# p-sawicki/entropy_coding

Hardware: AMD Instinct MI355X
Metric: Mbins/s encode+decode, intra QP32 synthetic bin buffers (higher is better)
Workload: dtype u32

## Files before the change

### entropy_coding_amd/csrc/cabac_kernels_v4.hip

```cpp
#include <cstdlib>
#include <type_traits>

#include "cabac_device.h"
#include "cabac_kernels.h"
#include "cabac_quad.h"

namespace cabac {


struct QuadEnc {
  uint64_t low;
  uint32_t range;
  int32_t pend;
  uint32_t buf;
  int32_t nbuf;
  uint32_t pos;
  uint8_t *dst;
  uint32_t cap;
};

__device__ __forceinline__ void quad_put_byte(QuadEnc &e, uint32_t byte, bool writer) {
  if (writer && e.pos < e.cap) e.dst[e.pos] = (uint8_t)byte;
  e.pos += 1;
}
// ... 117 lines not shown
    quad_put_byte(e, held, writer);
    held = 0;
    nb = 0;
  }
  const uint32_t n_bits = e.pos * 8u + nb;
  if (nb) quad_put_byte(e, held, writer);
  return n_bits;
}

template <class... Sets>
__global__ __launch_bounds__(64) void encode_kernel_v4(uint32_t n_sub, const cabac_substream_desc *__restrict__ desc,
                                                       const uint16_t *__restrict__ records, uint8_t *__restrict__ bytes,
                                                       cabac_substream_result *__restrict__ results, Sets... sets) {
  constexpr bool kSets = sizeof...(Sets) != 0;
  __shared__ uint32_t ctx[kQuadSubs * kQuadCtxStride];
  const uint32_t lane = threadIdx.x, row = lane >> 4, j = lane & 15u;
  const uint32_t sub = blockIdx.x * kQuadSubs + row;
  const QuadSetUse su = quad_set_use(sub, sub < n_sub, sets...);
  const bool live = sub < n_sub && !su.bad;
  const cabac_substream_desc d = desc[live ? sub : 0];
  const uint32_t n = live ? d.n_records : 0u;
  const uint16_t *rec = records + d.rec_offset;
  uint32_t *rctx = ctx + row * kQuadCtxStride;
  if constexpr (kSets) quad_ctx_load<true>(rctx, d.qp, d.init_id & 3u, j, 16u, su, sets...);
  else quad_ctx_init(rctx, d.qp, d.init_id & 3u, j);
  __syncthreads();

  QuadEnc e;
  e.low = 0;
  e.range = 510;
  e.pend = 0;
  e.buf = 0;
  e.nbuf = 0;
  e.pos = 0;
  e.dst = bytes + d.byte_offset;
  e.cap = live ? d.byte_capacity : 0u;
  const bool writer = live && j == 0;
  uint32_t bad = 0;

  uint32_t next_rec = j < n ? rec[j] : 0;
  for (uint32_t base = 0; __ballot(base < n) != 0; base += 16) {
    const uint32_t r = next_rec;
    const uint32_t info = quad_phase_a(r, base + j < n, lane, row, rctx, bad);
    const QuadEncInfo f = quad_unpack(info);
    {
      const uint32_t nxt = base + 16u + j;
      next_rec = nxt < n ? rec[nxt] : 0;
    }
    if (__ballot(info >> 12) == 0) quad_enc_steps<false, false>(f, e, writer, QuadPost());
    else quad_enc_steps<true, false>(f, e, writer, QuadPost());
  }

  const uint32_t n_bits = live ? quad_enc_finish(e, (d.init_id & CABAC_SUB_ALIGN_RBSP) != 0, writer, (d.init_id & CABAC_SUB_PROBE) != 0) : 0u;
  const uint64_t bad_mask = __ballot(bad != 0);
  const bool row_bad = ((bad_mask >> (row * 16u)) & 0xffffull) != 0;
  if (writer) {
    cabac_substream_result res;
    res.n_bits = n_bits;
    res.flags = (e.pos > e.cap ? CABAC_RES_OVERFLOW : 0u) | (row_bad ? CABAC_RES_BAD_RECORD : 0u);
    results[sub] = res;
  }
  if constexpr (kSets) {
    __syncthreads();
    quad_ctx_export(rctx, j, 16u, su, sets...);
    quad_bad_set_result(results, sub, j == 0, su);
  }
}

constexpr uint32_t kUnitSlots = 12;
constexpr uint32_t kUnitDump = 11;

template <int N>
__device__ __forceinline__ uint32_t row_shr(uint32_t v) {
  return (uint32_t)__builtin_amdgcn_update_dpp(0, (int)v, 0x110 + N, 0xf, 0xf, true);
}


struct QuadUnits {
  uint32_t m;
  uint64_t odd_rows;
  uint64_t store_lanes;
};

template <bool kHalfRows = false>
__device__ __forceinline__ QuadUnits quad_list_units(const QuadEnc &e, const uint32_t *plo, const uint32_t *phi,
                                                     const uint32_t *ppend, uint32_t row, uint32_t j, bool live,
                                                     uint32_t *list, uint32_t lane = 0) {
  const uint32_t c = (j & 3u) * kQuadSubs + row;
  const uint64_t low = ((uint64_t)phi[c] << 32) | plo[c];
  const uint32_t pend = ppend[c];
  const uint32_t nun = (pend >> 4) & neg_mask(j - 4u);
  const uint64_t v = low >> (9u + (pend & 15u));
  uint32_t incl = nun + row_shr<1>(nun);
  incl += row_shr<2>(incl);
  const uint32_t idx = incl - nun;
  const uint32_t first = (uint32_t)(v >> (((nun - 1u) & 1u) << 4));
  const uint32_t second = (uint32_t)v & 0xffffu;
  const uint32_t has1 = neg_mask(0u - nun);
  const uint32_t has2 = neg_mask(1u - nun);
  list[sel(has1, idx, kUnitDump)] = first;
  list[sel(has2, idx + 1u, kUnitDump)] = second;
  QuadUnits u;
  if (kHalfRows) u.m = (lane & 8u) ? row_bcast<11>(incl) : row_bcast<3>(incl);
  else u.m = row_bcast<3>(incl);
  const uint32_t room = e.cap - e.pos - 2u * u.m;
  const uint32_t rowodd = neg_mask(0u - u.m) & (neg_mask(0u - ((uint32_t)e.nbuf ^ 1u)) | neg_mask(room));
  u.odd_rows = __ballot(live && rowodd != 0);
  u.store_lanes = __ballot(live && j < u.m);
  return u;
}

__device__ __forceinline__ void quad_flush_list(QuadEnc &e, uint32_t m, const uint32_t *list, bool writer) {
  for (uint32_t k = 0; k < 8u && __ballot(k < m) != 0; k++) {
    if (k < m) quad_flush_lead(e, list[k], writer);
  }
}

__device__ __forceinline__ void quad_emit_units(QuadEnc &e, const QuadUnits &u, uint32_t j, const uint32_t *list,
                                                bool writer) {
  if (u.odd_rows != 0) return quad_flush_list(e, u.m, list, writer);
  const uint32_t act = neg_mask(j - u.m);
  const uint32_t jnz = neg_mask(0u - j);
  const uint32_t before = list[sel(act & jnz, j - 1u, kUnitDump)];
  const uint32_t mine = list[sel(act, j, kUnitDump)];
  const uint32_t last = list[sel(neg_mask(0u - u.m), u.m - 1u, kUnitDump)];
  const uint32_t x = (mine & 0x1ffffu) ^ 0xffffu;
  if (__ballot((act & neg_mask(x - 1u)) != 0) != 0) return quad_flush_list(e, u.m, list, writer);
  const uint32_t prev = sel(jnz, before & 0xffffu, e.buf);
  const uint32_t unit = prev + (mine >> 16);
  const uint32_t be = ((unit & 0xffu) << 8) | ((unit >> 8) & 0xffu);
  uint8_t *addr = e.dst + e.pos + 2u * j;
  uint64_t saved;
  asm volatile("s_mov_b64 %0, exec\n\ts_mov_b64 exec, %1\n\tglobal_store_short %2, %3, off\n\ts_mov_b64 exec, %0"
               : "=&s"(saved) : "s"(u.store_lanes), "v"(addr), "v"(be) : "memory");
  e.buf = sel(neg_mask(0u - u.m), last & 0xffffu, e.buf);
  e.pos += 2u * u.m;
}

#ifdef CABAC_V5_PROFILE
__device__ unsigned long long g_v5_prof[16];
#define V5_TICK(var) const unsigned long long var = __builtin_amdgcn_s_memtime()
#define V5_ADD(slot, t0, t1) \
  if (blockIdx.x == 0 && lane == 0) g_v5_prof[slot] += (t1) - (t0)
#else
#define V5_TICK(var)
#define V5_ADD(slot, t0, t1)
#endif
#ifndef CABAC_V5_STAMP_UNIT
#define CABAC_V5_STAMP_UNIT 0
#endif


struct QuadRngCap {
  uint32_t w[8];
};

template <int I, bool kAlign>
__device__ __forceinline__ void quad_rng_step(const QuadEncInfo &f, uint32_t &range, QuadRngCap &cap) {
  const uint32_t k = row_bcast<I>(f.k), c2 = row_bcast<I>(f.c2), lpsm = row_bcast<I>(f.lpsm);
  const uint32_t t = (__umul24((range >> 5) & 15u, k) + c2) >> 1;
  const uint32_t rm = range - t;
  const uint32_t x = sel(lpsm, t, rm);
  const uint32_t nb = (uint32_t)(__builtin_clz(x) - 23);
  range = x << nb;
  if (kAlign) range = sel(row_bcast<I>(f.alm), 256u, range);
  const uint32_t w = rm | (nb << 9);
  if (I & 1) cap.w[I >> 1] |= w << 16;
  else cap.w[I >> 1] = w;
}

struct QuadEncRow {
  uint32_t k[16], c2[16], lpsm[16];
};
template <int I, bool kAlign>
__device__ __forceinline__ void quad_rng_step_row(const QuadEncRow &u, const QuadEncInfo &f, uint32_t &range, QuadRngCap &cap) {
  const uint32_t t = (__umul24((range >> 5) & 15u, u.k[I]) + u.c2[I]) >> 1;
  const uint32_t rm = range - t;
  const uint32_t x = sel(u.lpsm[I], t, rm);
  const uint32_t nb = (uint32_t)(__builtin_clz(x) - 23);
  range = x << nb;
  if (kAlign) range = sel(row_bcast<I>(f.alm), 256u, range);
  const uint32_t w = rm | (nb << 9);
  if (I & 1) cap.w[I >> 1] |= w << 16;
  else cap.w[I >> 1] = w;
}
template <bool kAlign>
__device__ __forceinline__ void quad_rng_steps_row(const QuadEncRow &u, const QuadEncInfo &f, uint32_t &range, QuadRngCap &cap) {
#define QSTEP(I) quad_rng_step_row<I, kAlign>(u, f, range, cap)
  QSTEP(0); QSTEP(1); QSTEP(2); QSTEP(3); QSTEP(4); QSTEP(5); QSTEP(6); QSTEP(7);
  QSTEP(8); QSTEP(9); QSTEP(10); QSTEP(11); QSTEP(12); QSTEP(13); QSTEP(14); QSTEP(15);
#undef QSTEP
}

template <bool kAlign>
__device__ __forceinline__ void quad_rng_steps(const QuadEncInfo &f, uint32_t &range, QuadRngCap &cap) {
#define QSTEP(I) quad_rng_step<I, kAlign>(f, range, cap)
  QSTEP(0); QSTEP(1); QSTEP(2); QSTEP(3); QSTEP(4); QSTEP(5); QSTEP(6); QSTEP(7);
  QSTEP(8); QSTEP(9); QSTEP(10); QSTEP(11); QSTEP(12); QSTEP(13); QSTEP(14); QSTEP(15);
#undef QSTEP
}

__device__ __forceinline__ uint64_t shl64(uint32_t lo, uint32_t hi, uint32_t n) { return (((uint64_t)hi << 32) | lo) << n; }

__device__ __forceinline__ uint32_t quad_cap_mine(const QuadRngCap &cap, uint32_t j) {
  const uint32_t h = j >> 1;
  const uint32_t a0 = (h & 1u) ? cap.w[1] : cap.w[0], a1 = (h & 1u) ? cap.w[3] : cap.w[2], a2 = (h & 1u) ? cap.w[5] : cap.w[4],
                 a3 = (h & 1u) ? cap.w[7] : cap.w[6];
  const uint32_t b0 = (h & 2u) ? a1 : a0, b1 = (h & 2u) ? a3 : a2;
  const uint32_t pair = (h & 4u) ? b1 : b0;
  return ((j & 1u) ? pair >> 16 : pair) & 0xfffu;
}

__device__ __forceinline__ void quad_low_quads12(uint32_t w12, uint32_t info, uint32_t &v0, uint32_t &v1, uint32_t &s) {
  const uint32_t rm = w12 & 0x1ffu, nb = (w12 >> 9) & 7u;
  const uint32_t lpsm = bit_mask<9>(info), pem = bit_mask<11>(info), ep = (info >> 10) & 1u;
  const uint32_t term = ((rm & lpsm) << nb) | (rm & pem);
  s = nb + ep;
  uint64_t v = term;
  {
    const uint32_t p0 = row_shr<1>(term), ps = row_shr<1>(s);
    v = shl64(p0, 0u, s) + v;
    s += ps;
  }
  v0 = (uint32_t)v;
  {
    const uint32_t p0 = row_shr<2>(v0), ps = row_shr<2>(s);
    v = shl64(p0, 0u, s) + v;
    s += ps;
  }
// ... 225 lines not shown
    }
    if (n_iters != 0) {
#pragma unroll
      for (uint32_t h = 0; h < kSync; h++) list_step(kSync * (n_iters - 1u) + h);
    }
    if (j == 0u) {
      fin_acc[unit][row] = acc;
      fin_rem[unit][row] = rem;
    }
    __syncthreads();
    __syncthreads();
  } else {
    __builtin_amdgcn_s_setprio(CABAC_V6_PRIO_EMIT);
    QuadEnc e;
    e.low = 0;
    e.range = 0;
    e.pend = 0;
    e.buf = 0;
    e.nbuf = 0;
    e.pos = 0;
    e.dst = bytes + d.byte_offset;
    e.cap = live ? d.byte_capacity : 0u;
    const bool writer = live && j == 0;
    auto emit_step = [&](uint32_t step) {
      const uint32_t slot = step & (kRing - 1u);
      const uint32_t *list = unit_list[unit][slot][row];
      QuadUnits u;
      u.m = unit_count[unit][slot][row];
      const uint32_t room = e.cap - e.pos - 2u * u.m;
      const uint32_t rowodd = neg_mask(0u - u.m) & (neg_mask(0u - ((uint32_t)e.nbuf ^ 1u)) | neg_mask(room));
      u.odd_rows = __ballot(rowodd != 0);
      u.store_lanes = __ballot(live && j < u.m);
      quad_emit_units(e, u, j, list, writer);
    };
    __syncthreads();
    for (uint32_t it = 0; it < n_iters; it++) {
      V5_TICK(t0);
      if (it >= 2u) {
#pragma unroll
        for (uint32_t h = 0; h < kSync; h++) emit_step(kSync * (it - 2u) + h);
      }
      V5_TICK(t1);
      __syncthreads();
      V5_TICK(t2);
      if (unit == 0) V5_ADD(0, t0, t1);
      if (unit == 0) V5_ADD(12, t1, t2);
    }
    if (n_iters >= 2u) {
#pragma unroll
      for (uint32_t h = 0; h < kSync; h++) emit_step(kSync * (n_iters - 2u) + h);
    }
    __syncthreads();
    if (n_iters != 0) {
#pragma unroll
      for (uint32_t h = 0; h < kSync; h++) emit_step(kSync * (n_iters - 1u) + h);
    }
    __syncthreads();
    e.low = fin_acc[unit][row];
    e.pend = (int32_t)fin_rem[unit][row];
    const uint32_t n_bits = live ? quad_enc_finish(e, (d.init_id & CABAC_SUB_ALIGN_RBSP) != 0, writer, (d.init_id & CABAC_SUB_PROBE) != 0) : 0u;
    if (writer) {
      cabac_substream_result res;
      res.n_bits = n_bits;
      res.flags = (e.pos > e.cap ? CABAC_RES_OVERFLOW : 0u) | (((bad_rows[unit] >> row) & 1u) ? CABAC_RES_BAD_RECORD : 0u);
      results[sub] = res;
    }
    if constexpr (kSets) quad_bad_set_result(results, sub, j == 0, su);
  }
}

constexpr uint32_t kV7Pad = 20;
enum : uint32_t { kV7K = 0, kV7C2, kV7Lpsm, kV7Lp9, kV7Ep, kV7Fields };

__device__ __forceinline__ uint32_t lane_rng_step(uint32_t k, uint32_t c2, uint32_t lpsm, uint32_t &range) {
  const uint32_t t = (__umul24((range >> 5) & 15u, k) + c2) >> 1;
  const uint32_t rm = range - t;
  const uint32_t x = sel(lpsm, t, rm);
  const uint32_t nb = (uint32_t)(__builtin_clz(x) - 23);
  range = x << nb;
  return (nb << 9) + rm;
}

template <int U, class... Sets>
__global__ __launch_bounds__(64 * (U + 2 + (U + 1) / 2)) void encode_kernel_v7(uint32_t n_sub, const cabac_substream_desc *__restrict__ desc,
                                                                      const uint16_t *__restrict__ records,
                                                                      uint8_t *__restrict__ bytes,
                                                                      cabac_substream_result *__restrict__ results, Sets... sets) {
  constexpr bool kSets = sizeof...(Sets) != 0;
  constexpr uint32_t S = U * kQuadSubs;
  __shared__ uint32_t ctx_all[S * kQuadCtxStride];
  __shared__ __attribute__((aligned(16))) uint32_t fld[4][kV7Fields][S * kV7Pad];
  __shared__ __attribute__((aligned(16))) uint32_t wpost[2][(S + 1) * kV7Pad];
  __shared__ uint32_t post_lo[U][2][4 * kQuadSubs], post_hi[U][2][4 * kQuadSubs], post_pend[U][2][4 * kQuadSubs];
  __shared__ uint32_t fin_lo[S], fin_hi[S], fin_pend[S];
  __shared__ uint32_t unit_list[U][kQuadSubs][kUnitSlots];
  constexpr bool kKinds = U == 4;
  constexpr uint32_t kMatch = kKinds ? kMatchWordsCtx : kMatchWords;
  __shared__ uint32_t match_all[U][kMatch];
  __shared__ __attribute__((aligned(16))) uint4 kind_tab[kKinds ? kKindRows : 1];
  __shared__ uint2 rate_tab[kKinds ? 1 : 512];
  __shared__ uint32_t bad_rows[U];
  __shared__ uint32_t wg_max_n;
  const uint32_t wave = threadIdx.x >> 6, lane = threadIdx.x & 63u;
  if constexpr (kKinds) quad_kind_tab_init(kind_tab, threadIdx.x, blockDim.x);
  else quad_rate_tab_init(rate_tab, threadIdx.x, blockDim.x);
  constexpr bool kLdsMatch = true;
  for (uint32_t k = threadIdx.x; k < U * kMatch; k += blockDim.x) (&match_all[0][0])[k] = 0u;
  const uint32_t role_slot = U == 4 ? wave : (wave == 0 ? 0u : wave + 1u);
  const bool is_ctx = role_slot < 2u || (U == 4 && role_slot >= 6u);
  const bool is_chain = role_slot == 2u, is_low = role_slot == 3u;
  const bool is_out = !is_ctx && !is_chain && !is_low;
  const uint32_t ctx_unit = role_slot < 2u ? role_slot : role_slot - 4u;
  const uint32_t out_index = U == 4 ? role_slot - 4u : 0u;
  uint32_t row, j, unit, local;
  bool in_range = true;
  if (is_ctx) {
    row = lane >> 4;
    j = lane & 15u;
    unit = ctx_unit;
    local = unit * kQuadSubs + row;
  } else if (is_out) {
    const uint32_t g = out_index * 8u + (lane >> 3);
    in_range = g < S;
    local = min(g, S - 1u);
    unit = local >> 2;
    row = local & 3u;
    j = lane & 7u;
  } else {
    row = lane >> 4;
    j = lane & 15u;
    unit = 0;
    in_range = lane < S;
    local = min(lane, S - 1u);
  }
  const uint32_t sub = blockIdx.x * S + local;
  const QuadSetUse su = quad_set_use(sub, sub < n_sub, sets...);
  const bool in_batch = sub < n_sub && !su.bad;
  const bool live = in_batch && in_range;
  const cabac_substream_desc d = desc[in_batch ? sub : 0];
  const uint32_t n = in_batch ? d.n_records : 0u;

  if (threadIdx.x == 0) wg_max_n = 0;
  __syncthreads();
  atomicMax(&wg_max_n, n);
  __syncthreads();
  const uint32_t max_n = wg_max_n;
  const uint32_t n_steps = (max_n + 15u) >> 4;

  if (is_ctx) {
    const uint16_t *rec = records + d.rec_offset;
    uint32_t *rctx = ctx_all + local * kQuadCtxStride;
    if constexpr (kSets) quad_ctx_load<true>(rctx, d.qp, d.init_id & 3u, j, 16u, su, sets...);
    else quad_ctx_init(rctx, d.qp, d.init_id & 3u, j);
    uint32_t bad = 0;
    const uint16_t *rec_safe = n != 0 ? rec : reinterpret_cast<const uint16_t *>(desc);
    const uint32_t last_rec = n != 0 ? n - 1u : 0u;
    const uint32_t at = local * kV7Pad + j;
    auto post = [&](uint32_t slot, const QuadFields &f) {
      fld[slot][kV7K][at] = f.k;
      fld[slot][kV7C2][at] = f.c2;
      fld[slot][kV7Lpsm][at] = f.lpsm;
      fld[slot][kV7Lp9][at] = f.lp9;
      fld[slot][kV7Ep][at] = f.ep;
    };
    const uint32_t cur_rec = rec_safe[min(j, last_rec)];
    uint32_t next_rec = rec_safe[min(16u + j, last_rec)];
    uint32_t ahead1 = rec_safe[min(32u + j, last_rec)], ahead2 = rec_safe[min(48u + j, last_rec)], ahead3 = rec_safe[min(64u + j, last_rec)];
    post(0, quad_phase_fields<kLdsMatch, kKinds>(cur_rec, j < n, lane, row, rctx, bad, match_all[unit], rate_tab, kind_tab));
    __syncthreads();
    for (uint32_t k = 0; k < n_steps; k++) {
      const uint32_t base = 16u * k;
      const uint32_t r = next_rec;
      next_rec = ahead1;
      ahead1 = ahead2;
      ahead2 = ahead3;
      ahead3 = rec_safe[min(base + 80u + j, last_rec)];
      V5_TICK(t0);
      post((k + 1u) & 3u, quad_phase_fields<kLdsMatch, kKinds>(r, base + 16u + j < n, lane, row, rctx, bad, match_all[unit], rate_tab, kind_tab));
      V5_TICK(t1);
      __syncthreads();
      V5_TICK(t2);
      if (unit == CABAC_V5_STAMP_UNIT) V5_ADD(0, t0, t1);
      if (unit == CABAC_V5_STAMP_UNIT) V5_ADD(1, t1, t2);
    }
    const uint64_t bad_mask = __ballot(bad != 0);
    if (lane == 0) {
      uint32_t rows = 0;
      for (uint32_t q = 0; q < 4; q++) rows |= ((bad_mask >> (16u * q)) & 0xffffull) ? (1u << q) : 0u;
      bad_rows[unit] = rows;
    }
    if constexpr (kSets) {
      asm volatile("" ::: "memory");
      __builtin_amdgcn_wave_barrier();
      asm volatile("" ::: "memory");
      quad_ctx_export(rctx, j, 16u, su, sets...);
    }
    __syncthreads();
    __syncthreads();
  } else if (is_chain) {
    __builtin_amdgcn_s_setprio(3);
    uint32_t range = 510;
    __syncthreads();
    for (uint32_t k = 0; k < n_steps; k++) {
      V5_TICK(t0);
      const uint32_t slot = k & 3u;
      uint32_t kk[16], c2[16], lm[16], w[16];
#pragma unroll
      for (int q = 0; q < 4; q++) {
        lds_read4(&fld[slot][kV7K][local * kV7Pad], q, kk);
        lds_read4(&fld[slot][kV7C2][local * kV7Pad], q, c2);
        lds_read4(&fld[slot][kV7Lpsm][local * kV7Pad], q, lm);
      }
#pragma unroll
      for (int i = 0; i < 16; i++) w[i] = lane_rng_step(kk[i], c2[i], lm[i], range);
      uint4 *dst = reinterpret_cast<uint4 *>(&wpost[k & 1u][min(lane, S) * kV7Pad]);
#pragma unroll
      for (int i = 0; i < 4; i++) dst[i] = make_uint4(w[4 * i], w[4 * i + 1], w[4 * i + 2], w[4 * i + 3]);
      V5_TICK(t1);
      __syncthreads();
      V5_TICK(t2);
      V5_ADD(2, t0, t1);
      V5_ADD(3, t1, t2);
    }
    __syncthreads();
    __syncthreads();
  } else if (is_low) {
    uint64_t low = 0;
    uint32_t pend = 0;
    const uint32_t pu = local >> 2, pr = local & 3u;
    auto low_step = [&](uint32_t k) {
      const uint32_t slot = k & 3u;
      uint32_t w[16], lp9[16], ep[16];
#pragma unroll
      for (int q = 0; q < 4; q++) {
        lds_read4(&wpost[k & 1u][min(lane, S) * kV7Pad], q, w);
        lds_read4(&fld[slot][kV7Lp9][local * kV7Pad], q, lp9);
        lds_read4(&fld[slot][kV7Ep][local * kV7Pad], q, ep);
      }
#pragma unroll
      for (int i = 0; i < 16; i++) {
        const uint32_t nb = w[i] >> 9;
        const uint32_t term = (w[i] & lp9[i]) << nb;
        const uint32_t sh = nb + ep[i];
        low = (low << sh) + term;
        pend += sh;
        if ((i & 3) == 3) {
          const uint32_t c = (uint32_t)(i >> 2) * kQuadSubs + pr;
          post_lo[pu][k & 1u][c] = (uint32_t)low;
          post_hi[pu][k & 1u][c] = (uint32_t)(low >> 32);
          post_pend[pu][k & 1u][c] = pend;
          const uint32_t keep = pend & 15u;
          const uint32_t width = pend >= 16u ? 9u + keep : 63u;
          low &= ~(~0ull << width);
          pend = keep;
        }
      }
    };
    __syncthreads();
    for (uint32_t k = 0; k < n_steps; k++) {
      V5_TICK(t0);
      if (k != 0) low_step(k - 1u);
      V5_TICK(t1);
      __syncthreads();
      V5_TICK(t2);
      V5_ADD(4, t0, t1);
      V5_ADD(5, t1, t2);
    }
    if (n_steps != 0) low_step(n_steps - 1u);
    fin_lo[local] = (uint32_t)low;
    fin_hi[local] = (uint32_t)(low >> 32);
    fin_pend[local] = pend;
    __syncthreads();
    __syncthreads();
  } else {
    QuadEnc e;
    e.low = 0;
    e.range = 0;
    e.pend = 0;
    e.buf = 0;
    e.nbuf = 0;
    e.pos = 0;
    e.dst = bytes + d.byte_offset;
    e.cap = live ? d.byte_capacity : 0u;
    const bool writer = live && j == 0;
    uint32_t *list = unit_list[unit][row];
    QuadUnits units;
    units.m = 0;
    units.odd_rows = 0;
    units.store_lanes = 0;
    bool listed = false;
    auto list_step = [&](uint32_t k) {
      units = quad_list_units<true>(e, post_lo[unit][k & 1u], post_hi[unit][k & 1u], post_pend[unit][k & 1u], row, j, live, list, lane);
    };
    __syncthreads();
    for (uint32_t k = 0; k < n_steps; k++) {
      V5_TICK(t0);
      if (listed) quad_emit_units(e, units, j, list, writer);
      listed = k >= 2u;
      if (listed) list_step(k - 2u);
      V5_TICK(t1);
      __syncthreads();
      V5_TICK(t2);
      if (unit == CABAC_V5_STAMP_UNIT) V5_ADD(6, t0, t1);
      if (unit == CABAC_V5_STAMP_UNIT) V5_ADD(7, t1, t2);
    }
    if (listed) quad_emit_units(e, units, j, list, writer);
    if (n_steps >= 2u) {
      list_step(n_steps - 2u);
      quad_emit_units(e, units, j, list, writer);
    }
    __syncthreads();
    if (n_steps != 0) {
      list_step(n_steps - 1u);
      quad_emit_units(e, units, j, list, writer);
    }
    e.low = ((uint64_t)fin_hi[local] << 32) | fin_lo[local];
    e.pend = (int32_t)fin_pend[local];
    const uint32_t n_bits = live ? quad_enc_finish(e, (d.init_id & CABAC_SUB_ALIGN_RBSP) != 0, writer, (d.init_id & CABAC_SUB_PROBE) != 0) : 0u;
    if (writer) {
      cabac_substream_result res;
      res.n_bits = n_bits;
      res.flags = (e.pos > e.cap ? CABAC_RES_OVERFLOW : 0u) | (((bad_rows[unit] >> row) & 1u) ? CABAC_RES_BAD_RECORD : 0u);
      results[sub] = res;
    }
    if constexpr (kSets) quad_bad_set_result(results, sub, in_range && j == 0, su);
    __syncthreads();
  }
}


struct QuadDec {
  uint32_t hi, lo;
  uint32_t used;
  uint32_t range;
  uint32_t npos;
  uint32_t q_hi, q_lo;
  uint32_t *ring;
  uint32_t filled;
  uint32_t pf_data, pf_off, pf_mask;
  const uint8_t *src;
  uint32_t cap;
  const uint8_t *src_safe;
  uint32_t last_dword;
};

struct QuadDecInfo {
  uint32_t c2;
  uint32_t ep;
  uint32_t srmul;
  uint32_t ctxm;
  uint32_t ntrm;
  uint32_t alm;
  uint32_t key;
};

__device__ __forceinline__ void quad_dec_topup(QuadDec &w) {
  const uint64_t q = (((uint64_t)w.q_hi << 32) | w.q_lo) << (~w.npos & 31u);
  const uint32_t next32 = (uint32_t)(q >> 32);
  const uint32_t want = w.used;
  uint32_t add;
  asm("v_bfe_u32 %0, %1, %2, %3" : "=v"(add) : "v"(next32), "v"(32u - want), "v"(want));
  w.lo |= add;
  w.npos -= want;
  w.used = 0;
  const uint32_t *p = w.ring + ((w.npos >> 5) & 63u);
  w.q_lo = p[0];
  w.q_hi = p[1];
}

template <int L = 16>
__device__ __forceinline__ void quad_dec_stage_load(QuadDec &w, uint32_t j) {
  constexpr uint32_t kLanes = L > 16 ? 16u : (uint32_t)L;
  const uint32_t wanted = neg_mask(w.filled - (~w.npos >> 3) - 128u);
  w.pf_mask = L > 16 ? wanted & neg_mask(j - kLanes) : wanted;
  w.pf_off = w.filled + 4u * (j & (kLanes - 1u));
  w.pf_data = *reinterpret_cast<const uint32_t *>(w.src_safe + min(w.pf_off, w.last_dword));
  w.filled += (4u * kLanes) & wanted;
}
__device__ __forceinline__ void quad_dec_stage_store(QuadDec &w) {
  const uint32_t v = __builtin_bswap32(w.pf_data) & neg_mask(w.pf_off - w.cap);
  const uint32_t at = (w.pf_off >> 2) & 63u;
  w.ring[sel(w.pf_mask, 64u - at, 65u)] = v;
  w.ring[sel(w.pf_mask & neg_mask(at - 1u), 0u, 65u)] = v;
}

constexpr uint32_t kRingStride = 66;

// ... 593 lines not shown
  quad_ctx_load<true>(rctx, d.qp, d.init_id & 3u, j, 16u, su, cs);
  __syncthreads();

  uint32_t n_wave = n;
  n_wave = max(n_wave, (uint32_t)__shfl_xor((int)n_wave, 16));
  n_wave = max(n_wave, (uint32_t)__shfl_xor((int)n_wave, 32));
  const uint32_t max_n = (uint32_t)__builtin_amdgcn_readfirstlane((int)n_wave);
  const uint16_t *rec_safe = n != 0 ? rec : reinterpret_cast<const uint16_t *>(desc);
  const uint32_t last_rec = n != 0 ? n - 1u : 0u;
  uint32_t next_rec = rec_safe[min(j, last_rec)];
  uint32_t bad = 0;
  for (uint32_t base = 0; base < max_n; base += 16) {
    const uint32_t r = next_rec;
    next_rec = rec_safe[min(base + 16u + j, last_rec)];
    (void)quad_resolve<CABAC_REC_ALIGN, true>(r, base + j < n, lane, row, rctx, bad, match_all[wave]);
  }
  const uint64_t bad_mask = __ballot(bad != 0);
  asm volatile("" ::: "memory");
  __builtin_amdgcn_wave_barrier();
  asm volatile("" ::: "memory");
  quad_ctx_export(rctx, j, 16u, su, cs);
  if (sub < n_sub && j == 0 && flags != nullptr)
    flags[sub] = su.bad ? 0x40u : (((bad_mask >> (row * 16u)) & 0xffffull) ? CABAC_RES_BAD_RECORD : 0u);
}

hipError_t launch_ctx_advance(hipStream_t st, uint32_t n_sub, const cabac_substream_desc *desc, const uint16_t *records,
                              const CtxSets &sets, uint32_t *flags) {
  if (n_sub == 0) return hipSuccess;
  const uint32_t waves = (n_sub + kQuadSubs - 1) / kQuadSubs;
  if (waves >= 1024u) hipLaunchKernelGGL(ctx_advance_kernel<4>, dim3((waves + 3) / 4), dim3(256), 0, st, n_sub, desc, records, sets, flags);
  else hipLaunchKernelGGL(ctx_advance_kernel<1>, dim3(waves), dim3(64), 0, st, n_sub, desc, records, sets, flags);
  return hipGetLastError();
}

__global__ __launch_bounds__(256) void wpp_level_kernel(uint32_t first, uint32_t n, const cabac_substream_desc *__restrict__ desc,
                                                        const uint32_t *__restrict__ sync_from, const uint32_t *__restrict__ sync_at,
                                                        cabac_substream_desc *__restrict__ desc_out, uint32_t *__restrict__ start_out,
                                                        uint32_t *__restrict__ slot_out) {
  const uint32_t i = blockIdx.x * 256u + threadIdx.x;
  if (i >= n) return;
  const uint32_t s = first + i;
  cabac_substream_desc d = desc[s];
  d.n_records = min(sync_at[s], d.n_records);
  d.init_id &= 3u;
  desc_out[s] = d;
  const uint32_t from = sync_from[s];
  start_out[s] = (from == kNoSet || from < first) ? from : 0xfffffffeu;
  slot_out[s] = s;
}

hipError_t launch_wpp_level(hipStream_t st, uint32_t first, uint32_t n, const cabac_substream_desc *desc, const uint32_t *sync_from,
                            const uint32_t *sync_at, cabac_substream_desc *desc_out, uint32_t *start_out, uint32_t *slot_out) {
  if (n == 0) return hipSuccess;
  hipLaunchKernelGGL(wpp_level_kernel, dim3((n + 255u) / 256u), dim3(256), 0, st, first, n, desc, sync_from, sync_at, desc_out,
                     start_out, slot_out);
  return hipGetLastError();
}

hipError_t launch_encode_v4(hipStream_t st, uint32_t n_sub, const cabac_substream_desc *desc, const uint16_t *records,
                            uint8_t *bytes, cabac_substream_result *results, const CtxSets *sets) {
  const dim3 grid((n_sub + kQuadSubs - 1) / kQuadSubs);
  if (sets != nullptr) hipLaunchKernelGGL(encode_kernel_v4<CtxSets>, grid, dim3(64), 0, st, n_sub, desc, records, bytes, results, *sets);
  else hipLaunchKernelGGL(encode_kernel_v4<>, grid, dim3(64), 0, st, n_sub, desc, records, bytes, results);
  return hipGetLastError();
}

hipError_t launch_encode_v6(hipStream_t st, uint32_t n_sub, const cabac_substream_desc *desc, const uint16_t *records,
                            uint8_t *bytes, cabac_substream_result *results, uint32_t in_flight, const CtxSets *sets) {
  const uint32_t units = (n_sub + kQuadSubs - 1) / kQuadSubs;
  const uint32_t units_on_chip = (max(n_sub, in_flight) + kQuadSubs - 1) / kQuadSubs;
  if (sets != nullptr) {
    if (units_on_chip >= 1024u) hipLaunchKernelGGL((encode_kernel_v6<4, 1, CtxSets>), dim3((units + 3) / 4), dim3(1024), 0, st, n_sub, desc, records, bytes, results, *sets);
    else hipLaunchKernelGGL((encode_kernel_v6<1, 2, CtxSets>), dim3(units), dim3(256), 0, st, n_sub, desc, records, bytes, results, *sets);
    return hipGetLastError();
  }
  if (units_on_chip >= 1024u) hipLaunchKernelGGL((encode_kernel_v6<4, 1>), dim3((units + 3) / 4), dim3(1024), 0, st, n_sub, desc, records, bytes, results);
  else hipLaunchKernelGGL((encode_kernel_v6<1, 2>), dim3(units), dim3(256), 0, st, n_sub, desc, records, bytes, results);
  return hipGetLastError();
}

hipError_t launch_encode_v7(hipStream_t st, uint32_t n_sub, const cabac_substream_desc *desc, const uint16_t *records,
                            uint8_t *bytes, cabac_substream_result *results, uint32_t in_flight, const CtxSets *sets) {
  if (sets != nullptr) {
    if (max(n_sub, in_flight) >= 1024u) hipLaunchKernelGGL((encode_kernel_v7<4, CtxSets>), dim3((n_sub + 15) / 16), dim3(512), 0, st, n_sub, desc, records, bytes, results, *sets);
    else hipLaunchKernelGGL((encode_kernel_v7<1, CtxSets>), dim3((n_sub + 3) / 4), dim3(256), 0, st, n_sub, desc, records, bytes, results, *sets);
    return hipGetLastError();
  }
  if (max(n_sub, in_flight) >= 1024u) hipLaunchKernelGGL(encode_kernel_v7<4>, dim3((n_sub + 15) / 16), dim3(512), 0, st, n_sub, desc, records, bytes, results);
  else hipLaunchKernelGGL(encode_kernel_v7<1>, dim3((n_sub + 3) / 4), dim3(256), 0, st, n_sub, desc, records, bytes, results);
  return hipGetLastError();
}

__global__ __launch_bounds__(1024) void decode_select_kernel(uint32_t n_sub, const cabac_substream_desc *__restrict__ desc,
                                                             uint32_t threshold, uint32_t *__restrict__ select) {
  __shared__ unsigned long long sum_w[16];
  __shared__ uint32_t max_w[16];
  unsigned long long sum = 0;
  uint32_t mx = 0;
  for (uint32_t s = threadIdx.x; s < n_sub; s += 1024u) {
    const uint32_t n = desc[s].n_records;
    sum += n;
    mx = max(mx, n);
  }
  for (int d = 1; d < 64; d <<= 1) {
    sum += __shfl_xor(sum, d);
    mx = max(mx, (uint32_t)__shfl_xor((int)mx, d));
  }
  if ((threadIdx.x & 63u) == 0) {
    sum_w[threadIdx.x >> 6] = sum;
    max_w[threadIdx.x >> 6] = mx;
  }
  __syncthreads();
  if (threadIdx.x == 0) {
    for (int k = 1; k < 16; k++) {
      sum += sum_w[k];
      mx = max(mx, max_w[k]);
    }
    *select = (mx != 0 && sum >= (unsigned long long)threshold * mx) ? 1u : 0u;
  }
}

__global__ __launch_bounds__(1024) void decode_select_solo_kernel(uint32_t n_sub, const cabac_substream_desc *__restrict__ desc,
                                                                  uint32_t max_long, uint32_t *__restrict__ select) {
  __shared__ uint32_t red[16];
  __shared__ uint32_t longest;
  auto block_max = [&](uint32_t v) {
    for (int d = 1; d < 64; d <<= 1) v = max(v, (uint32_t)__shfl_xor((int)v, d));
    __syncthreads();
    if ((threadIdx.x & 63u) == 0) red[threadIdx.x >> 6] = v;
    __syncthreads();
    uint32_t m = 0;
    for (int k = 0; k < 16; k++) m = max(m, red[k]);
    return m;
  };
  uint32_t mx = 0;
  for (uint32_t s = threadIdx.x; s < n_sub; s += 1024u) mx = max(mx, desc[s].n_records);
  mx = block_max(mx);
  if (threadIdx.x == 0) longest = mx;
  __syncthreads();
  const uint32_t cut = longest >> 4;
  uint32_t past = 0;
  for (uint32_t s = threadIdx.x; s < n_sub; s += 1024u)
    if (desc[s].n_records > cut) past = s + 1u;
  past = block_max(past);
  if (threadIdx.x == 0) *select = (longest != 0u && past <= max_long) ? 2u : 0u;
}

static hipError_t launch_decode_v4_sets(hipStream_t st, uint32_t n_sub, const cabac_substream_desc *desc, const uint16_t *records,
                                        const uint8_t *bytes, uint8_t *bins, cabac_substream_result *results, uint32_t in_flight,
                                        int lanes_per_sub, uint32_t *select, const CtxSets &sets);

constexpr uint32_t kSoloUpTo = 1024;
constexpr uint32_t kSoloAskUpTo = 3072;
constexpr uint32_t kHexFrom = 9216;

hipError_t launch_decode_v4(hipStream_t st, uint32_t n_sub, const cabac_substream_desc *desc, const uint16_t *records,
                            const uint8_t *bytes, uint8_t *bins, cabac_substream_result *results, uint32_t in_flight, int lanes_per_sub,
                            uint32_t *select, const CtxSets *sets) {
  if (sets != nullptr) return launch_decode_v4_sets(st, n_sub, desc, records, bytes, bins, results, in_flight, lanes_per_sub, select, *sets);
  if (lanes_per_sub == 0) {
    if (max(n_sub, in_flight) <= kSoloUpTo) return launch_decode_v4(st, n_sub, desc, records, bytes, bins, results, in_flight, 64);
    if (select != nullptr && max(n_sub, in_flight) <= kSoloAskUpTo && in_flight <= n_sub) {
      hipLaunchKernelGGL(decode_select_solo_kernel, dim3(1), dim3(1024), 0, st, n_sub, desc, kSoloUpTo, select);
      hipLaunchKernelGGL((decode_kernel_v4<4, 64>), dim3((n_sub + 3u) / 4u), dim3(256), 0, st, n_sub, desc, records, bytes, bins, results, select, 2u);
      hipLaunchKernelGGL((decode_kernel_v4<4, 16>), dim3((n_sub + 15u) / 16u), dim3(256), 0, st, n_sub, desc, records, bytes, bins, results, select, 0u);
      return hipGetLastError();
    }
    if (max(n_sub, in_flight) < kHexFrom || select == nullptr) return launch_decode_v4(st, n_sub, desc, records, bytes, bins, results, in_flight, 16);
    const uint32_t thr = (uint32_t)((uint64_t)kHexFrom * n_sub / max(n_sub, in_flight));
    hipLaunchKernelGGL(decode_select_kernel, dim3(1), dim3(1024), 0, st, n_sub, desc, thr, select);
    hipLaunchKernelGGL((decode_kernel_v4<4, 4>), dim3((n_sub + 63u) / 64u), dim3(256), 0, st, n_sub, desc, records, bytes, bins, results, select, 1u);
// ... 61 lines not shown
```

Measured before the change: 88590.

## Rework v7 encoder wave roles: quad-lane low and output stages, drop a wave

Reassigns wave roles in encode_kernel_v7. The low-accumulation stage now spreads each substream across 4 lanes: it computes per-quad partial sums and chains carries between lanes with DPP, instead of one lane walking 16 symbols serially. The output stage likewise uses 4 lanes per substream, so a single out wave covers all 16 substreams. The U=4 block drops from 512 to 448 threads. The aim is to shorten the serial low-chain critical path and free a wave, at the cost of more cross-lane shuffles, a fallback flush when more than 4 units are pending, and an added waitcnt before the barrier.

```diff
diff --git a/entropy_coding_amd/csrc/cabac_kernels_v4.hip b/entropy_coding_amd/csrc/cabac_kernels_v4.hip
--- a/entropy_coding_amd/csrc/cabac_kernels_v4.hip
+++ b/entropy_coding_amd/csrc/cabac_kernels_v4.hip
@@ -223,17 +223,18 @@
   uint64_t store_lanes;
 };
 
-template <bool kHalfRows = false>
+template <int kLanes = 16>
 __device__ __forceinline__ QuadUnits quad_list_units(const QuadEnc &e, const uint32_t *plo, const uint32_t *phi,
                                                      const uint32_t *ppend, uint32_t row, uint32_t j, bool live,
-                                                     uint32_t *list, uint32_t lane = 0) {
+                                                     uint32_t *list) {
+  static_assert(kLanes == 16 || kLanes == 4, "a row or a quad per substream");
   const uint32_t c = (j & 3u) * kQuadSubs + row;
   const uint64_t low = ((uint64_t)phi[c] << 32) | plo[c];
   const uint32_t pend = ppend[c];
-  const uint32_t nun = (pend >> 4) & neg_mask(j - 4u);
+  const uint32_t nun = kLanes == 4 ? pend >> 4 : (pend >> 4) & neg_mask(j - 4u);
   const uint64_t v = low >> (9u + (pend & 15u));
-  uint32_t incl = nun + row_shr<1>(nun);
-  incl += row_shr<2>(incl);
+  uint32_t incl = nun + (kLanes == 4 ? row_shr<1>(nun) & neg_mask(0u - j) : row_shr<1>(nun));
+  incl += kLanes == 4 ? row_shr<2>(incl) & neg_mask(1u - j) : row_shr<2>(incl);
   const uint32_t idx = incl - nun;
   const uint32_t first = (uint32_t)(v >> (((nun - 1u) & 1u) << 4));
   const uint32_t second = (uint32_t)v & 0xffffu;
@@ -242,10 +243,10 @@
   list[sel(has1, idx, kUnitDump)] = first;
   list[sel(has2, idx + 1u, kUnitDump)] = second;
   QuadUnits u;
-  if (kHalfRows) u.m = (lane & 8u) ? row_bcast<11>(incl) : row_bcast<3>(incl);
-  else u.m = row_bcast<3>(incl);
+  u.m = group_bcast<kLanes, 3>(incl);
   const uint32_t room = e.cap - e.pos - 2u * u.m;
-  const uint32_t rowodd = neg_mask(0u - u.m) & (neg_mask(0u - ((uint32_t)e.nbuf ^ 1u)) | neg_mask(room));
+  uint32_t rowodd = neg_mask(0u - u.m) & (neg_mask(0u - ((uint32_t)e.nbuf ^ 1u)) | neg_mask(room));
+  if (kLanes == 4) rowodd |= neg_mask(4u - u.m);
   u.odd_rows = __ballot(live && rowodd != 0);
   u.store_lanes = __ballot(live && j < u.m);
   return u;
@@ -279,13 +280,16 @@
 }
 
 #ifdef CABAC_V5_PROFILE
-__device__ unsigned long long g_v5_prof[16];
+__device__ unsigned long long g_v5_prof[32];
 #define V5_TICK(var) const unsigned long long var = __builtin_amdgcn_s_memtime()
 #define V5_ADD(slot, t0, t1) \
   if (blockIdx.x == 0 && lane == 0) g_v5_prof[slot] += (t1) - (t0)
+#define V5_HW_ID(w) \
+  if (blockIdx.x == 0 && lane == 0) g_v5_prof[16 + (w)] = 0x100000000ull | (uint32_t)__builtin_amdgcn_s_getreg(4 | (31 << 11))
 #else
 #define V5_TICK(var)
 #define V5_ADD(slot, t0, t1)
+#define V5_HW_ID(w)
 #endif
 #ifndef CABAC_V5_STAMP_UNIT
 #define CABAC_V5_STAMP_UNIT 0
@@ -677,7 +681,7 @@
 }
 
 template <int U, class... Sets>
-__global__ __launch_bounds__(64 * (U + 2 + (U + 1) / 2)) void encode_kernel_v7(uint32_t n_sub, const cabac_substream_desc *__restrict__ desc,
+__global__ __launch_bounds__(64 * (U + 3)) void encode_kernel_v7(uint32_t n_sub, const cabac_substream_desc *__restrict__ desc,
                                                                       const uint16_t *__restrict__ records,
                                                                       uint8_t *__restrict__ bytes,
                                                                       cabac_substream_result *__restrict__ results, Sets... sets) {
@@ -697,36 +701,34 @@
   __shared__ uint32_t bad_rows[U];
   __shared__ uint32_t wg_max_n;
   const uint32_t wave = threadIdx.x >> 6, lane = threadIdx.x & 63u;
+  V5_HW_ID(wave);
   if constexpr (kKinds) quad_kind_tab_init(kind_tab, threadIdx.x, blockDim.x);
   else quad_rate_tab_init(rate_tab, threadIdx.x, blockDim.x);
   constexpr bool kLdsMatch = true;
   for (uint32_t k = threadIdx.x; k < U * kMatch; k += blockDim.x) (&match_all[0][0])[k] = 0u;
-  const uint32_t role_slot = U == 4 ? wave : (wave == 0 ? 0u : wave + 1u);
-  const bool is_ctx = role_slot < 2u || (U == 4 && role_slot >= 6u);
-  const bool is_chain = role_slot == 2u, is_low = role_slot == 3u;
-  const bool is_out = !is_ctx && !is_chain && !is_low;
-  const uint32_t ctx_unit = role_slot < 2u ? role_slot : role_slot - 4u;
-  const uint32_t out_index = U == 4 ? role_slot - 4u : 0u;
+  constexpr uint32_t kChainWave = U == 4 ? 3u : 1u, kLowWave = U == 4 ? 5u : 2u, kOutWave = U == 4 ? 6u : 3u;
+  const bool is_chain = wave == kChainWave, is_low = wave == kLowWave, is_out = wave == kOutWave;
+  const bool is_ctx = !is_chain && !is_low && !is_out;
   uint32_t row, j, unit, local;
   bool in_range = true;
   if (is_ctx) {
     row = lane >> 4;
     j = lane & 15u;
-    unit = ctx_unit;
+    unit = min(wave, U - 1u);
     local = unit * kQuadSubs + row;
-  } else if (is_out) {
-    const uint32_t g = out_index * 8u + (lane >> 3);
-    in_range = g < S;
-    local = min(g, S - 1u);
-    unit = local >> 2;
-    row = local & 3u;
-    j = lane & 7u;
-  } else {
+  } else if (is_chain) {
     row = lane >> 4;
     j = lane & 15u;
     unit = 0;
     in_range = lane < S;
     local = min(lane, S - 1u);
+  } else {
+    const uint32_t g = lane >> 2;
+    in_range = g < S;
+    local = min(g, S - 1u);
+    unit = local >> 2;
+    row = local & 3u;
+    j = lane & 3u;
   }
   const uint32_t sub = blockIdx.x * S + local;
   const QuadSetUse su = quad_set_use(sub, sub < n_sub, sets...);
@@ -822,34 +824,50 @@
   } else if (is_low) {
     uint64_t low = 0;
     uint32_t pend = 0;
-    const uint32_t pu = local >> 2, pr = local & 3u;
+    const uint32_t pu = local >> 2, pr = local & 3u, q = j;
+    auto quad_from_left = [](uint32_t v) {
+      return (uint32_t)__builtin_amdgcn_update_dpp(0, (int)v, 0x90, 0xf, 0xf, true);
+    };
     auto low_step = [&](uint32_t k) {
       const uint32_t slot = k & 3u;
-      uint32_t w[16], lp9[16], ep[16];
-#pragma unroll
-      for (int q = 0; q < 4; q++) {
-        lds_read4(&wpost[k & 1u][min(lane, S) * kV7Pad], q, w);
-        lds_read4(&fld[slot][kV7Lp9][local * kV7Pad], q, lp9);
-        lds_read4(&fld[slot][kV7Ep][local * kV7Pad], q, ep);
+      const uint4 w4 = reinterpret_cast<const uint4 *>(&wpost[k & 1u][local * kV7Pad])[q];
+      const uint4 l4 = reinterpret_cast<const uint4 *>(&fld[slot][kV7Lp9][local * kV7Pad])[q];
+      const uint4 e4 = reinterpret_cast<const uint4 *>(&fld[slot][kV7Ep][local * kV7Pad])[q];
+      const uint32_t w[4] = {w4.x, w4.y, w4.z, w4.w}, lp9[4] = {l4.x, l4.y, l4.z, l4.w}, ep[4] = {e4.x, e4.y, e4.z, e4.w};
+      uint32_t term[4], sh[4];
+#pragma unroll
+      for (int i = 0; i < 4; i++) {
+        const uint32_t nb = w[i] >> 9;
+        term[i] = (w[i] & lp9[i]) << nb;
+        sh[i] = nb + ep[i];
       }
-#pragma unroll
-      for (int i = 0; i < 16; i++) {
-        const uint32_t nb = w[i] >> 9;
-        const uint32_t term = (w[i] & lp9[i]) << nb;
-        const uint32_t sh = nb + ep[i];
-        low = (low << sh) + term;
-        pend += sh;
-        if ((i & 3) == 3) {
-          const uint32_t c = (uint32_t)(i >> 2) * kQuadSubs + pr;
-          post_lo[pu][k & 1u][c] = (uint32_t)low;
-          post_hi[pu][k & 1u][c] = (uint32_t)(low >> 32);
-          post_pend[pu][k & 1u][c] = pend;
-          const uint32_t keep = pend & 15u;
-          const uint32_t width = pend >= 16u ? 9u + keep : 63u;
-          low &= ~(~0ull << width);
-          pend = keep;
+      const uint32_t p01 = (term[0] << sh[1]) + term[1];
+      const uint64_t P = ((((uint64_t)p01 << sh[2]) + term[2]) << sh[3]) + term[3];
+      const uint32_t Ssum = sh[0] + sh[1] + sh[2] + sh[3];
+      uint64_t cut = 0, posted = 0;
+      uint32_t cut_pend = 0, posted_pend = 0;
+#pragma unroll
+      for (int r = 0; r < 4; r++) {
+        uint64_t in = low;
+        uint32_t in_pend = pend;
+        if (r != 0) {
+          const uint32_t lo = quad_from_left((uint32_t)cut), hi = quad_from_left((uint32_t)(cut >> 32)), pp = quad_from_left(cut_pend);
+          in = q == 0 ? low : ((uint64_t)hi << 32) | lo;
+          in_pend = q == 0 ? pend : pp;
         }
+        posted = (in << Ssum) + P;
+        posted_pend = in_pend + Ssum;
+        const uint32_t keep = posted_pend & 15u;
+        const uint32_t width = posted_pend >= 16u ? 9u + keep : 63u;
+        cut = posted & ~(~0ull << width);
+        cut_pend = keep;
       }
+      const uint32_t c = q * kQuadSubs + pr;
+      post_lo[pu][k & 1u][c] = (uint32_t)posted;
+      post_hi[pu][k & 1u][c] = (uint32_t)(posted >> 32);
+      post_pend[pu][k & 1u][c] = posted_pend;
+      low = ((uint64_t)group_bcast<4, 3>((uint32_t)(cut >> 32)) << 32) | group_bcast<4, 3>((uint32_t)cut);
+      pend = group_bcast<4, 3>(cut_pend);
     };
     __syncthreads();
     for (uint32_t k = 0; k < n_steps; k++) {
@@ -885,8 +903,9 @@
     units.store_lanes = 0;
     bool listed = false;
     auto list_step = [&](uint32_t k) {
-      units = quad_list_units<true>(e, post_lo[unit][k & 1u], post_hi[unit][k & 1u], post_pend[unit][k & 1u], row, j, live, list, lane);
+      units = quad_list_units<4>(e, post_lo[unit][k & 1u], post_hi[unit][k & 1u], post_pend[unit][k & 1u], row, j, live, list);
     };
+    __builtin_amdgcn_s_waitcnt(0x0f70);
     __syncthreads();
     for (uint32_t k = 0; k < n_steps; k++) {
       V5_TICK(t0);
@@ -896,8 +915,8 @@
       V5_TICK(t1);
       __syncthreads();
       V5_TICK(t2);
-      if (unit == CABAC_V5_STAMP_UNIT) V5_ADD(6, t0, t1);
-      if (unit == CABAC_V5_STAMP_UNIT) V5_ADD(7, t1, t2);
+      V5_ADD(6, t0, t1);
+      V5_ADD(7, t1, t2);
     }
     if (listed) quad_emit_units(e, units, j, list, writer);
     if (n_steps >= 2u) {
@@ -1657,11 +1676,11 @@
 hipError_t launch_encode_v7(hipStream_t st, uint32_t n_sub, const cabac_substream_desc *desc, const uint16_t *records,
                             uint8_t *bytes, cabac_substream_result *results, uint32_t in_flight, const CtxSets *sets) {
   if (sets != nullptr) {
-    if (max(n_sub, in_flight) >= 1024u) hipLaunchKernelGGL((encode_kernel_v7<4, CtxSets>), dim3((n_sub + 15) / 16), dim3(512), 0, st, n_sub, desc, records, bytes, results, *sets);
+    if (max(n_sub, in_flight) >= 1024u) hipLaunchKernelGGL((encode_kernel_v7<4, CtxSets>), dim3((n_sub + 15) / 16), dim3(448), 0, st, n_sub, desc, records, bytes, results, *sets);
     else hipLaunchKernelGGL((encode_kernel_v7<1, CtxSets>), dim3((n_sub + 3) / 4), dim3(256), 0, st, n_sub, desc, records, bytes, results, *sets);
     return hipGetLastError();
   }
-  if (max(n_sub, in_flight) >= 1024u) hipLaunchKernelGGL(encode_kernel_v7<4>, dim3((n_sub + 15) / 16), dim3(512), 0, st, n_sub, desc, records, bytes, results);
+  if (max(n_sub, in_flight) >= 1024u) hipLaunchKernelGGL(encode_kernel_v7<4>, dim3((n_sub + 15) / 16), dim3(448), 0, st, n_sub, desc, records, bytes, results);
   else hipLaunchKernelGGL(encode_kernel_v7<1>, dim3((n_sub + 3) / 4), dim3(256), 0, st, n_sub, desc, records, bytes, results);
   return hipGetLastError();
 }
```

Result: faster. 90360 (median of 6 runs) (+2.0%).
